# aosokin/os2d

Hardware: AMD Instinct MI355X
Metric: query-image-pairs/s (1280-px input, ResNet50, N-class) (higher is better)
Workload: dtype fftx3 (as fft; the per-bin complex GEMM on the fp16 MFMA with spectra split into fp16 hi+lo, 3 MFMAs per product, fp32 accumulate)

## Files before the change

os2d_amd/csrc/dft_mfma.h:

```cpp
#pragma once

#ifndef DFT_DEV
#error "the includer defines DFT_DEV, DFT_TID, DFT_BID, DFT_GRID, DFT_LDS, DFT_BARRIER, DFT_MFMA, DFT_SHFL_XOR, DFT_SHFL_XOR_U32, DFT_BALLOT, DFT_FLAG, DFT_FLAG_SET, DFT_RAISE, DFT_UNIFORM"
#endif

#ifndef DFT_MEMBER
#define DFT_MEMBER inline
#endif
#ifndef DFT_LANDED
#define DFT_LANDED(X)
#endif
#ifndef DFT_SWAP1
#define DFT_SWAP1(V) DFT_SHFL_XOR(V, 1)
#endif
#ifndef DFT_FWD_PREFETCH_AFTER
#define DFT_FWD_PREFETCH_AFTER 2
#endif
#ifndef DFT_INV_PREFETCH_AFTER
#define DFT_INV_PREFETCH_AFTER 2
#endif
#ifndef DFT_PIPE_REGA
#define DFT_PIPE_REGA 1
#endif
#ifndef DFT_PIPE_LDS
#define DFT_PIPE_LDS 1
#endif
#ifndef DFT_SCHED_FENCE
#define DFT_SCHED_FENCE()
#endif
#ifndef DFT_STREAM_STORE
#define DFT_STREAM_STORE(P, V) (*(P) = (V))
#endif
#ifndef DFT_STAMP
#define DFT_STAMP(K)
#define DFT_STAMP_BEGIN()
#define DFT_STAMP_END(BASE)
#endif

#include "tile_common.h"
#include "dft_plan.h"

namespace os2d_dft {

typedef float f32x4u __attribute__((ext_vector_type(4), aligned(4)));

DFT_DEV int dft_div(int x, unsigned magic) { return magic ? (int)(((unsigned long long)(unsigned)x * magic) >> 32) : x; }

DFT_DEV void dft_split4(float a, float b, float c, float d, u32x2* hi, u32x2* lo) {
  const f32x4 x = {a, b, c, d};
  const half4 h = __builtin_convertvector(x, half4);
  *hi = __builtin_bit_cast(u32x2, h);
#ifdef DFT_SPLIT_LO_PAIR
  u32x2 l;
  l[0] = DFT_SPLIT_LO_PAIR(a, b, (*hi)[0]);
  l[1] = DFT_SPLIT_LO_PAIR(c, d, (*hi)[1]);
  *lo = l;
#else
  const half4 l = __builtin_convertvector(x - __builtin_convertvector(h, f32x4), half4);
  *lo = __builtin_bit_cast(u32x2, l);
#endif
}

DFT_DEV half8 dft_frag(const u32x4* p) { return __builtin_bit_cast(half8, *p); }

DFT_DEV f32x16 dft_mma3(half8 ah, half8 al, half8 bh, half8 bl, f32x16 acc) {
  acc = DFT_MFMA(ah, bl, acc);
  acc = DFT_MFMA(al, bh, acc);
  acc = DFT_MFMA(ah, bh, acc);
  return acc;
}

template <int NT, int KS>
DFT_DEV void dft_product_rega(f32x16* acc, const half8* ah, const half8* al, int ksn, const u32x4* B, int bstride, int nt0,
                              int ntstep, int l31, int hw) {
  constexpr int KR = KS ? KS : DFT_KREG;
  half8 bh[2][NT], bl[2][NT];
#define DFT_REGA_READ(KSTEP, SET)                                                                                          \
  _Pragma("unroll") for (int j = 0; j < NT; ++j) {                                                                         \
    bh[SET][j] = dft_frag(B + (size_t)((2 * (KSTEP) + hw) * 2 + 0) * bstride + (nt0 + ntstep * j) * 32 + l31);             \
    bl[SET][j] = dft_frag(B + (size_t)((2 * (KSTEP) + hw) * 2 + 1) * bstride + (nt0 + ntstep * j) * 32 + l31);             \
  }
  if (DFT_PIPE_REGA) DFT_REGA_READ(0, 0)
#pragma unroll
  for (int ks = 0; ks < KR; ++ks) {
    if (KS || ks < ksn) {
      if (DFT_PIPE_REGA) {
        if (ks + 1 < KR && (KS || ks + 1 < ksn)) DFT_REGA_READ(ks + 1, (ks + 1) & 1)
        DFT_SCHED_FENCE();
      } else {
        DFT_REGA_READ(ks, ks & 1)
      }
#pragma unroll
      for (int j = 0; j < NT; ++j) acc[j] = dft_mma3(ah[ks], al[ks], bh[ks & 1][j], bl[ks & 1][j], acc[j]);
      if (DFT_PIPE_REGA) DFT_SCHED_FENCE();
    }
  }
#undef DFT_REGA_READ
}

template <int KS>
DFT_DEV void dft_product_rega_any(f32x16* acc, int ntiles, const half8* ah, const half8* al, int ksn, const u32x4* B, int bstride,
                                  int nt0, int ntstep, int l31, int hw) {
  if (ntiles == 3) dft_product_rega<3, KS>(acc, ah, al, ksn, B, bstride, nt0, ntstep, l31, hw);
  else if (ntiles == 2) dft_product_rega<2, KS>(acc, ah, al, ksn, B, bstride, nt0, ntstep, l31, hw);
  else if (ntiles == 1) dft_product_rega<1, KS>(acc, ah, al, ksn, B, bstride, nt0, ntstep, l31, hw);
}

template <int NT, bool SHARE, int NW, int PIPE_MODE>
DFT_DEV void dft_product_lds(f32x16* acc, int ks0, int ks1, const u32x4* A, int astride, const u32x4* B, int bstride, int t0, int mtn,
                             int l31, int hw) {
  constexpr int NA = SHARE ? 1 : NT;
  int tm[NT], tn[NT];
#pragma unroll
  for (int j = 0; j < NT; ++j) {
    const int t = t0 + NW * j;
    tn[j] = t / mtn;
    tm[j] = t - tn[j] * mtn;
  }
  half8 ah[2][NA], al[2][NA], bh[2][NT], bl[2][NT];
#define DFT_LDS_READ(KSTEP, SET)                                                                                           \
  {                                                                                                                        \
    const int kc_ = (KSTEP) < ks1 ? (KSTEP) : ks1 - 1;                                                                     \
    _Pragma("unroll") for (int j = 0; j < NA; ++j) {                                                                       \
      ah[SET][j] = dft_frag(A + (size_t)((2 * kc_ + hw) * 2 + 0) * astride + tm[j] * 32 + l31);                            \
      al[SET][j] = dft_frag(A + (size_t)((2 * kc_ + hw) * 2 + 1) * astride + tm[j] * 32 + l31);                            \
    }                                                                                                                      \
    _Pragma("unroll") for (int j = 0; j < NT; ++j) {                                                                       \
      bh[SET][j] = dft_frag(B + (size_t)((2 * kc_ + hw) * 2 + 0) * bstride + tn[j] * 32 + l31);                            \
      bl[SET][j] = dft_frag(B + (size_t)((2 * kc_ + hw) * 2 + 1) * bstride + tn[j] * 32 + l31);                            \
    }                                                                                                                      \
  }
#define DFT_LDS_MMA(SET)                                                                                                   \
  DFT_SCHED_FENCE();                                                                                                       \
  _Pragma("unroll") for (int j = 0; j < NT; ++j)                                                                           \
    acc[j] = dft_mma3(ah[SET][SHARE ? 0 : j], al[SET][SHARE ? 0 : j], bh[SET][j], bl[SET][j], acc[j]);                    \
  DFT_SCHED_FENCE();
  if (ks0 >= ks1) return;
  constexpr bool PIPE = PIPE_MODE == 2 || (PIPE_MODE == 1 && SHARE);
  if (!PIPE) {
    for (int ks = ks0; ks < ks1; ++ks) {
      DFT_LDS_READ(ks, 0)
      _Pragma("unroll") for (int j = 0; j < NT; ++j)
        acc[j] = dft_mma3(ah[0][SHARE ? 0 : j], al[0][SHARE ? 0 : j], bh[0][j], bl[0][j], acc[j]);
    }
    return;
  }
  DFT_LDS_READ(ks0, 0)
  int ks = ks0;
  for (; ks + 1 < ks1; ks += 2) {
    DFT_LDS_READ(ks + 1, 1)
    DFT_LDS_MMA(0)
    DFT_LDS_READ(ks + 2, 0)
    DFT_LDS_MMA(1)
  }
  if (ks < ks1) {
    DFT_LDS_MMA(0)
  }
#undef DFT_LDS_READ
#undef DFT_LDS_MMA
}

template <int NW, int PIPE_MODE>
DFT_DEV void dft_product_lds_any(f32x16* acc, int ntiles, int ks0, int ks1, const u32x4* A, int astride, const u32x4* B, int bstride,
                                 int t0, int mtn, int l31, int hw) {
  const bool share = mtn == NW;
  if (ntiles == 3) {
    if (share) dft_product_lds<3, true, NW, PIPE_MODE>(acc, ks0, ks1, A, astride, B, bstride, t0, mtn, l31, hw);
    else dft_product_lds<3, false, NW, PIPE_MODE>(acc, ks0, ks1, A, astride, B, bstride, t0, mtn, l31, hw);
  } else if (ntiles == 2) {
    if (share) dft_product_lds<2, true, NW, PIPE_MODE>(acc, ks0, ks1, A, astride, B, bstride, t0, mtn, l31, hw);
    else dft_product_lds<2, false, NW, PIPE_MODE>(acc, ks0, ks1, A, astride, B, bstride, t0, mtn, l31, hw);
  } else if (ntiles == 1) {
    dft_product_lds<1, true, NW, PIPE_MODE>(acc, ks0, ks1, A, astride, B, bstride, t0, mtn, l31, hw);
  }
}

DFT_DEV void dft_matrix_unit(int which, int unit, int P, int Q, const double* twP, const double* twQ, u32x4* out) {
  const int V = Q / 2 + 1;
  const bool r2 = which == 1 && dft_radix2(P);
  if (r2 && unit >= DFT_R2_MATU) {
    const int u = 2 * (unit - DFT_R2_MATU);
    u32x4 o;
    for (int t = 0; t < 4; ++t) o[t] = __builtin_bit_cast(unsigned, (float)twP[2 * u + t]);
    *out = o;
    return;
  }
  const int tws = r2 ? 2 : 1;
  if (r2) P /= 2;
  const int Pp = dft_round_up(P, 8);
  int cols, kidx, hl, col;
  double vals[8];
  if (which == 0) cols = dft_round_up(2 * V, 32);
  else if (which == 1 || which == 2) cols = dft_round_up(2 * P, 32);
  else cols = dft_round_up(Q, 32);
  col = unit % cols;
  hl = (unit / cols) & 1;
  kidx = unit / (2 * cols);
  for (int t = 0; t < 8; ++t) {
    const int k = kidx * 8 + t;
    double x = 0.0;
    if (which == 0) {
      const int v = col >> 1, ri = col & 1;
      if (k < Q && v < V) x = twQ[2 * (int)(((long long)v * k) % Q) + ri] * DFT_SCALE_F;
    } else if (r2) {
      const int h = 8 * (2 * (kidx >> 1) + (t >> 2)) + 4 * (kidx & 1) + (t & 3), u = col & 31;
      if (kidx < 4) {
        const int a = (int)(((long long)u * h) % P) * tws;
        x = (col < 32 ? twP[2 * a] : -twP[2 * a + 1]) * DFT_SCALE_F;
      }
    } else if (which == 1) {
      const int ri = k / Pp, h = k - ri * Pp, u = col >> 1, ro = col & 1;
      if (h < P && u < P && ri < 2) {
        const int a = (int)(((long long)u * h) % P) * tws;
        const double c = twP[2 * a], s = -twP[2 * a + 1];
        x = (ro == 0 ? (ri == 0 ? c : s) : (ri == 0 ? -s : c)) * DFT_SCALE_F;
      }
    } else if (which == 2) {
      const int ri = k / Pp, u = k - ri * Pp, h = col >> 1, ro = col & 1;
      if (u < P && h < P && ri < 2) {
        const int a = (int)(((long long)u * h) % P);
        const double c = twP[2 * a], s = -twP[2 * a + 1];
        x = (ro == 0 ? (ri == 0 ? c : -s) : (ri == 0 ? s : c)) * DFT_SCALE_F;
      }
    } else {
      const int v = k >> 1, ri = k & 1;
      if (v < V && col < Q) {
        const double a = (v == 0 || 2 * v == Q) ? 1.0 : 2.0;
        x = a * twQ[2 * (int)(((long long)v * col) % Q) + ri] * DFT_SCALE_GQ;
      }
    }
    vals[t] = x;
  }
  unsigned w[4];
  for (int t = 0; t < 4; ++t) {
    unsigned short b[2];
    for (int e = 0; e < 2; ++e) {
      const double x = vals[2 * t + e];
      const _Float16 h = (_Float16)x;
      const _Float16 r = hl == 0 ? h : (_Float16)(x - (double)h);
      b[e] = __builtin_bit_cast(unsigned short, r);
    }
    w[t] = (unsigned)b[0] | ((unsigned)b[1] << 16);
  }
  u32x4 o;
  o[0] = w[0];
  o[1] = w[1];
  o[2] = w[2];
  o[3] = w[3];
  *out = o;
}

template <bool TILED, bool FAST, int G, int NW, int KS2 = 0>
DFT_DEV void dft_forward_body(const float* corr,
                              const float* invn,
                              float* X,
                              const u32x4* FqT, const u32x4* Fp2, const DftPlan& pl, int C, int Cpad, int NBT, int iters) {
  constexpr int THR = NW * 64;
  constexpr bool ALDS = G == 8;
  constexpr bool R2 = !ALDS && KS2 == DFT_R2_KS;
  unsigned char* smem = DFT_LDS;
  const int tid = DFT_TID, lane = tid & 63, l31 = lane & 31, hw = lane >> 5;
  const int wv = DFT_UNIFORM(tid >> 6);
  const int P = pl.P, V = pl.V, Pp = pl.Pp, Wk = pl.Wk, N1 = pl.N1, Mx = pl.Mx, N2 = pl.N2, LH = pl.LH, LW = pl.LW, W = pl.W, H = pl.H;
  const int MxS = dft_pitch_x(pl), N2S = dft_pitch_n2(pl);
  const int CG = (C + G - 1) / G, HW = H * W;
  const bool unit_norm = invn == nullptr;
  u32x4* ldsF = reinterpret_cast<u32x4*>(smem);
  u32x4* ldsU = reinterpret_cast<u32x4*>(smem + pl.lds_const);
  unsigned char* ldsUb = smem + pl.lds_const;
  const int nF = dft_lds_fqt(pl);
  for (int i = tid; i < nF; i += THR) ldsF[i] = FqT[i];
  const unsigned char* ldsTw = dft_lds_tail_ptr(smem, pl) + DFT_TAIL_TW;
  if (R2 && tid < DFT_R2_TWU) reinterpret_cast<u32x4*>(dft_lds_tail_ptr(smem, pl) + DFT_TAIL_TW)[tid] = Fp2[DFT_R2_MATU + tid];
  u32x4* ldsP = ldsF + nF;
  if (ALDS)
    for (int i = tid; i < dft_lds_rowop(Pp, pl.M2); i += THR) ldsP[i] = Fp2[i];

  const int mt1n = Mx / 32, nt1n = N1 / 32, nt2n = N2 / 32, mt2n = pl.M2 / 32;
  const int ks1n = Wk / 16, ks2n = 2 * Pp / 16;
  const int mt2 = wv & 3;
  constexpr int KR2 = R2 ? 4 : KS2 ? KS2 : DFT_KREG;
  half8 fp2h[KR2], fp2l[KR2];
  if (R2) {
#pragma unroll
    for (int f = 0; f < KR2; ++f) {
      fp2h[f] = dft_frag(Fp2 + ((size_t)((2 * (f & 1) + hw) * 2 + 0)) * 64 + (f >> 1) * 32 + l31);
      fp2l[f] = dft_frag(Fp2 + ((size_t)((2 * (f & 1) + hw) * 2 + 1)) * 64 + (f >> 1) * 32 + l31);
    }
  } else if (!ALDS) {
#pragma unroll
    for (int ks = 0; ks < KR2; ++ks) {
      const int kc = ks < ks2n ? ks : 0, mc = mt2 < mt2n ? mt2 : 0;
      fp2h[ks] = dft_frag(Fp2 + ((size_t)((2 * kc + hw) * 2 + 0)) * pl.M2 + mc * 32 + l31);
      fp2l[ks] = dft_frag(Fp2 + ((size_t)((2 * kc + hw) * 2 + 1)) * pl.M2 + mc * 32 + l31);
    }
  }
  if (!ALDS) {
#pragma unroll
    for (int ks = 0; ks < KR2; ++ks) {
// ... 216 lines not shown

      const int XS = dft_pitch_xs(P, G);
#pragma unroll
      for (int j = 0; j < DFT_ACC_TILES; ++j) {
        if (un[j] < 0) continue;
        const int n2 = un[j] * 32 + l31;
        const int img = dft_div(n2, pl.inv_v), v = n2 - img * V;
#pragma unroll
        for (int q = 0; q < 4; ++q) {
          const int u0 = (um[j] * 32 + 8 * q + 4 * hw) >> 1;
          if (img < G && u0 < P) {
            const float sc = DFT_SCALE_XOUT;
            f32x4 o;
            o[0] = xc[j][4 * q] * sc;
            o[1] = xc[j][4 * q + 1] * sc;
            o[2] = xc[j][4 * q + 2] * sc;
            o[3] = xc[j][4 * q + 3] * sc;
            *reinterpret_cast<f32x4*>(ldsUb + (size_t)v * XS + (u0 >> 2) * (G * 32) + img * 32 + (u0 & 3) * 8) = o;
          }
        }
      }
      DFT_BARRIER();
      DFT_STAMP(4)
    }

    {
      const int XS = dft_pitch_xs(P, G);
      const int per_v = (P / 4) * (G * 2), npieces = V * per_v;
      size_t qstride;
      float* dstbase = X + dft_spectra_pair0(pr_, NBT, pl.NBINS / 4, Cpad, &qstride) + (size_t)c0_ * 8;
      if (R2) {
        constexpr int per_h = (DFT_R2_P / 8) * (G * 2);
        for (int i = tl; i < V * per_h; i += THR) {
          const int v = i / per_h, rem = i - v * per_h;
          const int uq = rem / (2 * G), jj = rem - uq * (2 * G);
          const unsigned char* src = ldsUb + (size_t)v * XS + uq * (G * 32) + jj * 16;
          const f32x4 e = *reinterpret_cast<const f32x4*>(src);
          const f32x4 o = *reinterpret_cast<const f32x4*>(src + (DFT_R2_P / 8) * (G * 32));
          const f32x4 w = *reinterpret_cast<const f32x4*>(ldsTw + (4 * uq + 2 * (jj & 1)) * 8);
          f32x4 t;
          t[0] = w[0] * o[0] - w[1] * o[1];
          t[1] = w[0] * o[1] + w[1] * o[0];
          t[2] = w[2] * o[2] - w[3] * o[3];
          t[3] = w[2] * o[3] + w[3] * o[2];
          float* dst = dstbase + (size_t)(v * (P / 4) + uq) * qstride + jj * 4;
          DFT_STREAM_STORE(reinterpret_cast<f32x4*>(dst), e + t);
          DFT_STREAM_STORE(reinterpret_cast<f32x4*>(dst + (size_t)(DFT_R2_P / 8) * qstride), e - t);
        }
      } else
      for (int i = tl; i < npieces; i += THR) {
        const int v = dft_div(i, pl.inv_pq), rem = i - v * per_v;
        const int uq = rem / (2 * G), jj = rem - uq * (2 * G);
        const f32x4 val = *reinterpret_cast<const f32x4*>(ldsUb + (size_t)v * XS + uq * (G * 32) + jj * 16);
        DFT_STREAM_STORE(reinterpret_cast<f32x4*>(dstbase + (size_t)(v * (P / 4) + uq) * qstride + jj * 4), val);
      }
      const int qpad0 = (P * V) / 4, qpad1 = pl.NBINS / 4;
      for (int i = tl; i < (qpad1 - qpad0) * 2 * G; i += THR)
        *reinterpret_cast<f32x4*>(dstbase + (size_t)(qpad0 + i / (2 * G)) * qstride + (i % (2 * G)) * 4) = f32x4{0.f, 0.f, 0.f, 0.f};
    }
    DFT_BARRIER();
    DFT_STAMP(5)
  }
  DFT_STAMP_END(0)
#undef DFT_FWD_ITER
#undef DFT_FWD_POS
#undef DFT_FWD_PREFETCH
#undef DFT_FWD_PREFETCH_SLOTS
}

template <bool TILED, int KSA = 0, int G = DFT_G>
DFT_DEV void dft_inverse_body(const float* Y,
                              const float* bp,
                              int MTP, unsigned char* out,
                              const u32x4* E2, const u32x4* Gq, const DftPlan& pl, int Cout, int NBT, int PLANE, int Ws,
                              int BASE, int iters, DFT_FLAG bad_flag, int zero_borders) {
  unsigned char* smem = DFT_LDS;
  const int tid = DFT_TID, lane = tid & 63, l31 = lane & 31, hw = lane >> 5;
  const int wv = DFT_UNIFORM(tid >> 6);
  const int P = pl.P, V = pl.V, Pp = pl.Pp, N2 = pl.N2, MB = pl.MB, KB = pl.KB, NBo = pl.NBo, H = pl.H, W = pl.W;
  const int N2S = dft_pitch_n2(pl), MBS = dft_pitch_tt(pl);
  const int OG = Cout / G;
  constexpr bool ALDS = G == 8;
  constexpr int LG = G == 8 ? 3 : 2;
  u32x4* ldsG = reinterpret_cast<u32x4*>(smem);
  u32x4* ldsU = reinterpret_cast<u32x4*>(smem + pl.lds_const);
  unsigned char* ldsUb = smem + pl.lds_const;
  float* smaxw = reinterpret_cast<float*>(dft_lds_tail_ptr(smem, pl) + DFT_TAIL_MAX);
  const int nG = dft_lds_gq(pl), NQ = dft_round_up(pl.Q, 32);
  for (int i = tid; i < nG; i += DFT_THR) {
    const int kh = i / NBo, n = i - kh * NBo;
    ldsG[i] = Gq[(size_t)kh * NQ + n];
  }
  const int MAfull = dft_round_up(2 * P, 32);
  u32x4* ldsE = ldsG + nG;
  if (ALDS)
    for (int i = tid; i < dft_lds_rowop(Pp, MAfull); i += DFT_THR) ldsE[i] = E2[i];

  const int mtAn = pl.MA / 32, ntAn = N2 / 32, ksAn = 2 * Pp / 16;
  const int mtBn = MB / 32, ntBn = NBo / 32, ksBn = KB / 16;
  const int mtA = wv & 3;
  constexpr int KRA = KSA ? KSA : DFT_KREG;
  half8 e2h[KRA], e2l[KRA];
  if (!ALDS) {
#pragma unroll
    for (int ks = 0; ks < KRA; ++ks) {
      const int kc = ks < ksAn ? ks : 0, mc = mtA < mtAn ? mtA : 0;
      e2h[ks] = dft_frag(E2 + ((size_t)((2 * kc + hw) * 2 + 0)) * MAfull + mc * 32 + l31);
      e2l[ks] = dft_frag(E2 + ((size_t)((2 * kc + hw) * 2 + 1)) * MAfull + mc * 32 + l31);
    }
#pragma unroll
    for (int ks = 0; ks < KRA; ++ks) {
      DFT_LANDED(e2h[ks]);
      DFT_LANDED(e2l[ks]);
    }
  }

  constexpr int NITEM = DFT_ITEMS;
  const int uoct = Pp / 8, nitem = G * V * uoct;
  f32x4 py[NITEM][4];
#define DFT_INV_PREFETCH(IT, TID) DFT_INV_PREFETCH_ITEMS(IT, TID, 0, NITEM)
#define DFT_INV_PREFETCH_ITEMS(IT, TID, S0, S1)                                             \
  {                                                                                         \
    const int pr_ = dft_div((IT), pl.inv_og), og_ = (IT)-pr_ * OG;                          \
    size_t qstride;                                                                         \
    const float* src_ = Y + dft_spectra_pair0(pr_, NBT, pl.NBINS / 4, Cout, &qstride) + (size_t)og_ * G * 8; \
    _Pragma("unroll") for (int s = (S0); s < (S1); ++s) {                                   \
      const int e_ = (TID) + s * DFT_THR;                                                   \
      const int ec_ = e_ < nitem ? e_ : 0;                                                  \
      const int pimg_ = ec_ & (G - 1), prest_ = ec_ >> LG;                                  \
      const int pv_ = dft_div(prest_, pl.inv_kg), puo_ = prest_ - pv_ * (Pp / 8);           \
      const int q0_ = pv_ * (P / 4) + 2 * puo_;                                             \
      const bool ptwo_ = 8 * puo_ + 4 < P;                                                  \
      const float* p0_ = src_ + (size_t)q0_ * qstride + pimg_ * 8;                          \
      const float* p1_ = src_ + (size_t)(ptwo_ ? q0_ + 1 : q0_) * qstride + pimg_ * 8;      \
      py[s][0] = *reinterpret_cast<const f32x4*>(p0_);                                     \
      py[s][1] = *reinterpret_cast<const f32x4*>(p0_ + 4);                                 \
      py[s][2] = *reinterpret_cast<const f32x4*>(p1_);                                     \
      py[s][3] = *reinterpret_cast<const f32x4*>(p1_ + 4);                                 \
    }                                                                                       \
  }
#define DFT_INV_ITEM(E)                                                                     \
  const int img_ = (E) & (G - 1), rest_ = (E) >> LG;                                        \
  const int v_ = dft_div(rest_, pl.inv_kg), uo_ = rest_ - v_ * uoct;                        \
  const bool two_ = 8 * uo_ + 4 < P;
#define DFT_INV_MAXIMA(TID)                                                                 \
  {                                                                                         \
    float m = 0.f;                                                                          \
    _Pragma("unroll") for (int s = 0; s < NITEM; ++s)                                       \
      if ((TID) + s * DFT_THR < nitem) {                                                    \
        DFT_INV_ITEM((TID) + s * DFT_THR)                                                   \
        (void)img_;                                                                         \
        (void)v_;                                                                           \
        (void)uo_;                                                                          \
        _Pragma("unroll") for (int k = 0; k < 4; ++k)                                       \
          if (k < 2 || two_) {                                                              \
            _Pragma("unroll") for (int e = 0; e < 4; ++e) m = fmaxf(m, fabsf(py[s][k][e])); \
          }                                                                                 \
      }                                                                                     \
    if (G == 4) m = fmaxf(m, DFT_SHFL_XOR(m, 4));                                           \
    m = fmaxf(m, DFT_SHFL_XOR(m, 8));                                                       \
    m = fmaxf(m, DFT_SHFL_XOR(m, 16));                                                      \
    m = fmaxf(m, DFT_SHFL_XOR(m, 32));                                                      \
    if (lane < G) smaxw[wv * G + lane] = m;                                                 \
  }
  bool bad = false;
  const int first = (DFT_GRID & 7) == 0 ? (DFT_BID & 7) * (DFT_GRID >> 3) + (DFT_BID >> 3) : DFT_BID;
  if (first < iters) {
    DFT_INV_PREFETCH(first, tid)
    DFT_INV_MAXIMA(tid)
  }
  DFT_BARRIER();

  DFT_STAMP_BEGIN()
  for (int it = first; it < iters; it += DFT_GRID) {
    int tl = tid;
#ifndef OS2D_HOST_EMU
    asm volatile("" : "+v"(tl));
#endif
    const int lane = tl & 63, l31 = lane & 31, hw = lane >> 5;
    const int pr = dft_div(it, pl.inv_og), og = it - pr * OG;
    const int nb = TILED ? dft_div(pr, pl.inv_t) : pr, tile = TILED ? pr - nb * pl.T : 0;
    const int ty = TILED ? dft_div(tile, pl.inv_tx) : 0, tx = TILED ? tile - ty * pl.TX : 0;
    const int y0 = TILED ? ty * pl.TH : 0, x0 = TILED ? tx * pl.TW : 0, oy = TILED ? pl.oy : 0, ox = TILED ? pl.ox : 0;
    const int TH_ = TILED ? pl.TH : H, TW_ = TILED ? pl.TW : W;
    const int o0 = og * G;

    DFT_STAMP(0)
    float simg = 1.f, cinv[4] = {0.f, 0.f, 0.f, 0.f};
    {
#pragma unroll
      for (int g = 0; g < G; ++g) {
        float m = 0.f;
#pragma unroll
        for (int w = 0; w < DFT_WAVES; ++w) m = fmaxf(m, smaxw[w * G + g]);
        int E = (int)((__builtin_bit_cast(unsigned, m) >> 23) & 0xffu) - 127;
        if (!(m > 0.f) || E < -100) E = -100;
        if (E > 100) E = 100;
        const float s = __builtin_bit_cast(float, (unsigned)(DFT_EY - E + 127) << 23);
        const float sinv = __builtin_bit_cast(float, (unsigned)(E - DFT_EY + 127) << 23);
        if (g == (tl & (G - 1))) simg = s;
        const float ci = sinv * __builtin_bit_cast(float, (unsigned)(pl.eT - DFT_EGQ + 127) << 23) / (float)(P * pl.Q);
        if (G == 4 || (g >> 2) == hw) cinv[g & 3] = ci;
      }
    }
#pragma unroll
    for (int s = 0; s < NITEM; ++s) {
      const int e = tl + s * DFT_THR;
      if (e < nitem) {
        DFT_INV_ITEM(e)
        const int img = img_, v = v_, uo = uo_;
        const bool two = two_;
        float re[8], im[8];
#pragma unroll
        for (int k = 0; k < 4; ++k) {
          const bool ok = k < 2 || two;
          re[2 * k] = ok ? py[s][k][0] * simg : 0.f;
          im[2 * k] = ok ? py[s][k][1] * simg : 0.f;
          re[2 * k + 1] = ok ? py[s][k][2] * simg : 0.f;
          im[2 * k + 1] = ok ? py[s][k][3] * simg : 0.f;
        }
        u32x2 h0, l0, h1, l1;
        u32x4 t;
        const size_t n = (size_t)img * V + v;
        dft_split4(re[0], re[1], re[2], re[3], &h0, &l0);
        dft_split4(re[4], re[5], re[6], re[7], &h1, &l1);
        t[0] = h0[0], t[1] = h0[1], t[2] = h1[0], t[3] = h1[1];
        ldsU[(size_t)((uo)*2 + 0) * N2S + n] = t;
        t[0] = l0[0], t[1] = l0[1], t[2] = l1[0], t[3] = l1[1];
        ldsU[(size_t)((uo)*2 + 1) * N2S + n] = t;
        dft_split4(im[0], im[1], im[2], im[3], &h0, &l0);
        dft_split4(im[4], im[5], im[6], im[7], &h1, &l1);
        t[0] = h0[0], t[1] = h0[1], t[2] = h1[0], t[3] = h1[1];
        ldsU[(size_t)((uoct + uo) * 2 + 0) * N2S + n] = t;
        t[0] = l0[0], t[1] = l0[1], t[2] = l1[0], t[3] = l1[1];
        ldsU[(size_t)((uoct + uo) * 2 + 1) * N2S + n] = t;
      }
    }
    DFT_BARRIER();
    DFT_STAMP(1)

    f32x16 ta[DFT_ACC_TILES];
    int an[DFT_ACC_TILES], am[DFT_ACC_TILES];
    int ntaw = 0;
#pragma unroll
    for (int j = 0; j < DFT_ACC_TILES; ++j) {
      const int t = wv + DFT_WAVES * j;
      const int nt = ALDS ? t / mtAn : (wv >> 2) + 2 * j;
      const bool mine = ALDS ? t < mtAn * ntAn : (nt < ntAn && mtA < mtAn);
      an[j] = mine ? nt : -1;
      am[j] = ALDS ? t - nt * mtAn : mtA;
      ntaw += mine ? 1 : 0;
#pragma unroll
      for (int r = 0; r < 16; ++r) ta[j][r] = 0.f;
    }
    const int itn = it + DFT_GRID < iters ? it + DFT_GRID : it;
    {
      if (ALDS) {
        dft_product_lds_any<DFT_WAVES, DFT_PIPE_LDS ? 1 : 0>(ta, ntaw, 0, ksAn, ldsE, MAfull, ldsU, N2S, wv, mtAn, l31, hw);
        DFT_INV_PREFETCH_ITEMS(itn, tl, 0, NITEM)
      } else if (DFT_INV_PREFETCH_AFTER == 1 || (DFT_INV_PREFETCH_AFTER == 2 && KSA > 0 && KSA <= 6)) {
        dft_product_rega_any<KSA>(ta, ntaw, e2h, e2l, ksAn, ldsU, N2S, wv >> 2, 2, l31, hw);
        DFT_INV_PREFETCH_ITEMS(itn, tl, 0, NITEM)
      } else {
        DFT_INV_PREFETCH_ITEMS(itn, tl, 0, NITEM)
        dft_product_rega_any<KSA>(ta, ntaw, e2h, e2l, ksAn, ldsU, N2S, wv >> 2, 2, l31, hw);
      }
    }
    DFT_BARRIER();
    DFT_STAMP(2)

    {
      const float sc = __builtin_bit_cast(float, (unsigned)(127 - DFT_EF - pl.eT) << 23);
#pragma unroll
      for (int j = 0; j < DFT_ACC_TILES; ++j) {
        if (an[j] < 0) continue;
        const int n = an[j] * 32 + l31;
        const int img = dft_div(n, pl.inv_v), v = n - img * V;
        if (img >= G) continue;
#pragma unroll
        for (int q = 0; q < 4; ++q) {
          const int h0 = (am[j] * 32 + 8 * q + 4 * hw) >> 1;
          u32x2 hi, lo;
          dft_split4(ta[j][4 * q] * sc, ta[j][4 * q + 1] * sc, ta[j][4 * q + 2] * sc, ta[j][4 * q + 3] * sc, &hi, &lo);
          unsigned char* d0 = ldsUb + ((size_t)((v >> 2) * 2) * MBS + (size_t)h0 * G + img) * 16 + (v & 3) * 4;
          *reinterpret_cast<unsigned*>(d0) = hi[0];
          *reinterpret_cast<unsigned*>(d0 + (size_t)MBS * 16) = lo[0];
          *reinterpret_cast<unsigned*>(d0 + G * 16) = hi[1];
          *reinterpret_cast<unsigned*>(d0 + G * 16 + (size_t)MBS * 16) = lo[1];
        }
      }
      for (int v = V; v < KB / 2; ++v)
        for (int m = tl; m < MB; m += DFT_THR) {
          unsigned char* d0 = ldsUb + ((size_t)((v >> 2) * 2) * MBS + m) * 16 + (v & 3) * 4;
          *reinterpret_cast<unsigned*>(d0) = 0u;
          *reinterpret_cast<unsigned*>(d0 + (size_t)MBS * 16) = 0u;
        }
    }
    DFT_BARRIER();
    DFT_STAMP(3)

    f32x16 yc[DFT_ACC_TILES];
    int bm[DFT_ACC_TILES], bn[DFT_ACC_TILES];
    int ntbw = 0;
#pragma unroll
    for (int j = 0; j < DFT_ACC_TILES; ++j) {
      const int t = wv + DFT_WAVES * j;
      const bool mine = t < mtBn * ntBn;
      bn[j] = mine ? t / mtBn : 0;
      bm[j] = mine ? t - bn[j] * mtBn : -1;
      ntbw += mine ? 1 : 0;
#pragma unroll
      for (int r = 0; r < 16; ++r) yc[j][r] = 0.f;
    }
    dft_product_lds_any<DFT_WAVES, DFT_PIPE_LDS ? 1 : 0>(yc, ntbw, 0, ksBn, ldsU, MBS, ldsG, NBo, wv, mtBn, l31, hw);
    DFT_INV_MAXIMA(tl)
    DFT_STAMP(4)

    {
      const bool planes = zero_borders == DFT_OUT_PLANES;
      float bias[4], osc[4];
#pragma unroll
      for (int g = 0; g < 4; ++g) {
        bias[g] = bp[o0 + (G == 8 ? 4 * hw : 0) + g];
        osc[g] = bp[2 * MTP + o0 + (G == 8 ? 4 * hw : 0) + g];
      }
      const int grp = o0 >> 3, slot = o0 & 7;
      unsigned char* hi_unit = out + (((size_t)nb * ((Cout + 7) >> 3) + grp) * 2 + 0) * (size_t)PLANE * 16 + slot * 2;
      unsigned char* lo_unit = out + (((size_t)nb * ((Cout + 7) >> 3) + grp) * 2 + 1) * (size_t)PLANE * 16 + slot * 2;
      if (zero_borders == DFT_OUT_SHB_BORDERS && (!TILED || tile == 0)) {
        const int rows = H * (Ws - W), tail0 = BASE + H * Ws, npad = BASE + rows + (PLANE - tail0);
        for (int k = tl; k < npad; k += DFT_THR) {
          int cell;
          if (k < BASE) cell = k;
          else if (k < BASE + rows) {
            const int jj = k - BASE, hr = jj / (Ws - W);
            cell = BASE + hr * Ws + W + (jj - hr * (Ws - W));
          } else cell = tail0 + (k - BASE - rows);
          if (G == 8) {
            *reinterpret_cast<u32x4*>(hi_unit + (size_t)cell * 16) = u32x4{0u, 0u, 0u, 0u};
            *reinterpret_cast<u32x4*>(lo_unit + (size_t)cell * 16) = u32x4{0u, 0u, 0u, 0u};
          } else {
            *reinterpret_cast<u32x2*>(hi_unit + (size_t)cell * 16) = u32x2{0u, 0u};
            *reinterpret_cast<u32x2*>(lo_unit + (size_t)cell * 16) = u32x2{0u, 0u};
          }
        }
      }
#pragma unroll
      for (int j = 0; j < DFT_ACC_TILES; ++j) {
        if (bm[j] < 0) continue;
        const int wwin = bn[j] * 32 + l31, tw = wwin - ox;
#pragma unroll
        for (int q = 0; q < 4; ++q) {
          const int hwin = G == 8 ? bm[j] * 4 + q : (bm[j] * 32 + 8 * q + 4 * hw) >> 2, th = hwin - oy;
          const int h = y0 + th, w = x0 + tw;
          const bool inside = th >= 0 && th < TH_ && tw >= 0 && tw < TW_ && h < H && w < W;
          if (G == 8 || inside) {
            float t[4];
#pragma unroll
            for (int g = 0; g < 4; ++g) {
              const float pre = yc[j][4 * q + g] * cinv[g] + bias[g];
              t[g] = fmaxf(pre, 0.f) * osc[g];
              if (inside && (!(fabsf(t[g]) <= 65504.f) || pre != pre)) bad = true;
            }
            if (planes) {
              if (inside) {
                float* dst = reinterpret_cast<float*>(out) + ((size_t)nb * Cout + o0 + (G == 8 ? 4 * hw : 0)) * ((size_t)H * W) + (size_t)h * W + w;
#pragma unroll
                for (int g = 0; g < 4; ++g) dst[(size_t)g * H * W] = t[g] * DFT_SCALE_PLANES;
              }
              continue;
            }
            u32x2 hi, lo;
            dft_split4(t[0], t[1], t[2], t[3], &hi, &lo);
            const size_t off = ((size_t)BASE + (size_t)h * Ws + w) * 16;
// ... 30 lines not shown
```

os2d_amd/csrc/dft_plan.h:

```cpp
#pragma once

#include <stddef.h>
#include <stdlib.h>

#ifndef DFT_HD
#define DFT_HD static inline
#endif

namespace os2d_dft {

constexpr int DFT_THR = 512, DFT_WAVES = 8;
constexpr int DFT_G = 4;
constexpr int DFT_MAXP = 64;
constexpr int DFT_MAXV = 48;
constexpr int DFT_MAXWK = 96;
constexpr int DFT_KREG = 8;
constexpr int DFT_LDS_MAX = 160 * 1024;
constexpr int DFT_OUT_SHB = 0, DFT_OUT_SHB_BORDERS = 1, DFT_OUT_PLANES = 2;

constexpr int DFT_ACC_TILES = 3;
constexpr int DFT_SLOTS_G4 = 3, DFT_SLOTS_G8 = 2;
constexpr int DFT_ITEMS = 3;

constexpr int DFT_EX = 15;
constexpr int DFT_EF = 14;
constexpr int DFT_EGQ = 13;
constexpr int DFT_ER = 8;
constexpr int DFT_EY = 13;
constexpr double dft_pow2(int e) { return e >= 0 ? (double)(1 << e) : 1.0 / (double)(1 << -e); }
constexpr float DFT_SCALE_X = (float)dft_pow2(DFT_EX);
constexpr double DFT_SCALE_F = dft_pow2(DFT_EF), DFT_SCALE_GQ = dft_pow2(DFT_EGQ);
constexpr float DFT_SCALE_R = (float)dft_pow2(DFT_ER - DFT_EX - DFT_EF);
constexpr float DFT_SCALE_XOUT = (float)dft_pow2(-(DFT_ER + DFT_EF));
constexpr float DFT_SCALE_PLANES = (float)dft_pow2(-DFT_EX);

struct DftPlan {
  int H, W;
  int P, Q, V, NBINS;
  int T, TY, TX, TH, TW;
  int oy, ox;
  int LH, LW;
  int RH;
  int Pp;
  int Wk;
  int N1;
  int M2;
  int Mx;
  int N2;
  int MA;
  int MB;
  int KB;
  int NBo;
  int G;
  int eT;
  int fast;
  unsigned inv_cg, inv_t, inv_tx, inv_c4, inv_v, inv_pq, inv_og, inv_kg, inv_pp;
  int lds_const, lds_union, lds_total;
};

DFT_HD constexpr int dft_round_up(int x, int m) { return (x + m - 1) / m * m; }
DFT_HD unsigned dft_magic(unsigned d) { return d > 1 ? (unsigned)(((1ull << 32) + d - 1) / d) : 0u; }

DFT_HD int dft_units_fqt(int P, int Q) { return (dft_round_up(Q, 16) / 8) * 2 * dft_round_up(Q + 2, 32); }
constexpr int DFT_R2_P = 64, DFT_R2_MATU = 8 * 2 * 64, DFT_R2_TWU = 16;
DFT_HD bool dft_radix2(int P) { return P == DFT_R2_P; }
DFT_HD int dft_units_fp2(int P, int Q) {
  return dft_radix2(P) ? DFT_R2_MATU + DFT_R2_TWU : (2 * dft_round_up(P, 8) / 8) * 2 * dft_round_up(2 * P, 32);
}
DFT_HD int dft_units_e2(int P, int Q) { return (2 * dft_round_up(P, 8) / 8) * 2 * dft_round_up(2 * P, 32); }
DFT_HD int dft_units_gq(int P, int Q) { return (dft_round_up(Q + 2, 16) / 8) * 2 * dft_round_up(Q, 32); }
DFT_HD size_t dft_matrices_units(int P, int Q) {
  return (size_t)dft_units_fqt(P, Q) + dft_units_fp2(P, Q) + dft_units_e2(P, Q) + dft_units_gq(P, Q);
}

DFT_HD int dft_lds_units(int k, int pitch) { return (k / 8) * 2 * pitch; }
DFT_HD int dft_lds_fqt(const DftPlan& pl) { return dft_lds_units(pl.Wk, pl.N1); }
DFT_HD int dft_lds_gq(const DftPlan& pl) { return dft_lds_units(pl.KB, pl.NBo); }
DFT_HD int dft_lds_rowop(int Pp, int rows) { return dft_lds_units(2 * Pp, rows); }
DFT_HD int dft_pitch_x(const DftPlan& pl) { return pl.Mx + 1; }
DFT_HD int dft_pitch_n2(const DftPlan& pl) { return pl.N2 + 1; }
DFT_HD int dft_pitch_tt(const DftPlan& pl) { return pl.MB + 1; }
DFT_HD int dft_pitch_xs(int P, int G) { return P * 8 * G + 16; }
DFT_HD int dft_lds_x_bytes(const DftPlan& pl) { return dft_lds_units(pl.Wk, dft_pitch_x(pl)) * 16; }
DFT_HD int dft_lds_n2_bytes(const DftPlan& pl) { return dft_lds_units(2 * pl.Pp, dft_pitch_n2(pl)) * 16; }
DFT_HD int dft_lds_xs_bytes(const DftPlan& pl, int G) { return pl.V * dft_pitch_xs(pl.P, G); }
DFT_HD int dft_lds_tt_bytes(const DftPlan& pl) { return dft_lds_units(pl.KB, dft_pitch_tt(pl)) * 16; }
constexpr int DFT_TAIL_BYTES = 1024;
constexpr int DFT_TAIL_MAX = 0, DFT_TAIL_TW = 512;
constexpr int dft_tail_max_bytes(int G) { return DFT_WAVES * G * 4; }
static_assert(DFT_TAIL_MAX + dft_tail_max_bytes(8) <= DFT_TAIL_TW, "the maxima of 8 images end in front of the twiddles");
static_assert(DFT_TAIL_TW + DFT_R2_TWU * 16 <= DFT_TAIL_BYTES, "the twiddles end inside the tail");
DFT_HD int dft_lds_tail(const DftPlan& pl) { return pl.lds_const + pl.lds_union; }
DFT_HD unsigned char* dft_lds_tail_ptr(unsigned char* smem, const DftPlan& pl) { return smem + pl.lds_const + pl.lds_union; }

struct DftCounts {
  int t1, t2, tA, tB;
  int rows2, cols2;
  int npos, nitem;
};
DFT_HD DftCounts dft_plan_counts(const DftPlan& pl) {
  DftCounts c;
  c.t1 = (pl.Mx / 32) * (pl.N1 / 32);
  c.t2 = (pl.M2 / 32) * (pl.N2 / 32);
  c.tA = (pl.MA / 32) * (pl.N2 / 32);
  c.tB = (pl.MB / 32) * (pl.NBo / 32);
  c.rows2 = (pl.M2 > pl.MA ? pl.M2 : pl.MA) / 32;
  c.cols2 = pl.N2 / 32;
  c.npos = pl.Pp * (pl.Wk / 4);
  c.nitem = pl.G * pl.V * (pl.Pp / 8);
  return c;
}
DFT_HD bool dft_capacity_ok(const DftPlan& pl) {
  const DftCounts c = dft_plan_counts(pl);
  const int tiles = DFT_WAVES * DFT_ACC_TILES;
  if (c.t1 > tiles || c.tB > tiles || c.nitem > DFT_ITEMS * DFT_THR) return false;
  if (pl.G == 8) return c.t2 <= tiles && c.tA <= tiles && c.npos <= DFT_SLOTS_G8 * DFT_THR;
  return c.rows2 <= 4 && c.cols2 <= (DFT_WAVES / 4) * DFT_ACC_TILES && c.npos <= DFT_SLOTS_G4 * DFT_THR;
}
static_assert(dft_round_up(DFT_G * DFT_MAXP, 32) / 32 <= DFT_WAVES && dft_round_up(2 * DFT_MAXV, 32) / 32 <= DFT_ACC_TILES,
              "step 1: at most 8 x 3 tiles");
static_assert(dft_round_up(2 * DFT_MAXP, 32) / 32 <= 4 && dft_round_up(DFT_G * DFT_MAXV, 32) / 32 <= (DFT_WAVES / 4) * DFT_ACC_TILES,
              "step 2 / step A: at most 4 row tiles, 6 column tiles reached as (wave >> 2) + 2 j");
static_assert(DFT_G * (dft_round_up(2 * DFT_MAXP, 32) / 2) / 32 <= DFT_WAVES && dft_round_up(DFT_MAXWK, 32) / 32 <= DFT_ACC_TILES,
              "step B: at most 8 x 3 tiles");
static_assert(dft_round_up(DFT_MAXP, 8) * (DFT_MAXWK / 4) <= DFT_SLOTS_G4 * DFT_THR, "window positions: at most 64 * 24");
static_assert(DFT_G * DFT_MAXV * (dft_round_up(DFT_MAXP, 8) / 8) <= DFT_ITEMS * DFT_THR, "spectrum items: at most 4 * 48 * 8");
static_assert(2 * dft_round_up(DFT_MAXP, 8) / 16 <= DFT_KREG, "k-steps of the register-resident operand");

static inline bool dft_plan_transform(int LH, int LW, int RH, int ncols, int minP, int minQ, int G, DftPlan* pl) {
  pl->G = G;
  pl->P = dft_round_up(minP, 4);
  if (pl->P == 60) pl->P = DFT_R2_P;
  pl->Q = dft_round_up(minQ, 2);
  pl->V = pl->Q / 2 + 1;
  pl->NBINS = dft_round_up(pl->P * pl->V, 8);
  pl->LH = LH;
  pl->LW = LW;
  pl->RH = RH;
  pl->Pp = dft_round_up(pl->P, 8);
  pl->Wk = dft_round_up(LW, 16);
  pl->N1 = dft_round_up(2 * pl->V, 32);
  pl->M2 = dft_round_up(2 * pl->P, 32);
  pl->Mx = dft_round_up(G * pl->Pp, 32);
  pl->N2 = dft_round_up(G * pl->V, 32);
  pl->MA = dft_round_up(2 * RH, 32);
  pl->MB = G * (pl->MA / 2);
  pl->KB = dft_round_up(2 * pl->V, 16);
  pl->NBo = dft_round_up(ncols, 32);
  int e = 0;
  while ((1 << e) < pl->P) ++e;
  pl->eT = e + 1;
  if (pl->P > DFT_MAXP || pl->V > DFT_MAXV || pl->Wk > DFT_MAXWK || LH > pl->P || LW > pl->Q || RH > pl->P) return false;
// ... 103 lines not shown
```

Measured before the change: 51830.

## Use radix-2 even/odd split for the P=64 inverse DFT stage

For P=64 the inverse stage now does a radix-2 decimation instead of a dense complex DFT GEMM. It multiplies even- and odd-indexed halves by a half-size 32-point DFT matrix held in registers, then combines them with twiddles staged in LDS to write both output halves. This is meant to cut MFMA work and the register footprint of the E2 matrix, at the cost of more epilogue arithmetic and a new matrix layout. It also zeroes the padded spectrum rows with wide vector stores instead of per-word stores.

```diff
diff --git a/os2d_amd/csrc/dft_mfma.h b/os2d_amd/csrc/dft_mfma.h
--- a/os2d_amd/csrc/dft_mfma.h
+++ b/os2d_amd/csrc/dft_mfma.h
@@ -18,6 +18,9 @@
 #endif
 #ifndef DFT_INV_PREFETCH_AFTER
 #define DFT_INV_PREFETCH_AFTER 2
+#endif
+#ifndef DFT_INV_ZERO_WIDE
+#define DFT_INV_ZERO_WIDE 1
 #endif
 #ifndef DFT_PIPE_REGA
 #define DFT_PIPE_REGA 1
@@ -106,6 +109,35 @@
   else if (ntiles == 1) dft_product_rega<1, KS>(acc, ah, al, ksn, B, bstride, nt0, ntstep, l31, hw);
 }
 
+template <int NT>
+DFT_DEV void dft_product_rega_eo(f32x16* e, f32x16* o, const half8* ah, const half8* al, const u32x4* B, int bstride, int nt0,
+                                 int ntstep, int l31, int hw) {
+  constexpr int KR = DFT_R2_KS / 2;
+  half8 bh[2][2][NT], bl[2][2][NT];
+#define DFT_EO_READ(KSTEP, SET)                                                                                            \
+  _Pragma("unroll") for (int p = 0; p < 2; ++p) _Pragma("unroll") for (int j = 0; j < NT; ++j) {                           \
+    bh[SET][p][j] = dft_frag(B + (size_t)((2 * ((KSTEP) + KR * p) + hw) * 2 + 0) * bstride + (nt0 + ntstep * j) * 32 + l31); \
+    bl[SET][p][j] = dft_frag(B + (size_t)((2 * ((KSTEP) + KR * p) + hw) * 2 + 1) * bstride + (nt0 + ntstep * j) * 32 + l31); \
+  }
+  if (DFT_PIPE_REGA) DFT_EO_READ(0, 0)
+#pragma unroll
+  for (int ks = 0; ks < KR; ++ks) {
+    if (DFT_PIPE_REGA) {
+      if (ks + 1 < KR) DFT_EO_READ(ks + 1, (ks + 1) & 1)
+      DFT_SCHED_FENCE();
+    } else {
+      DFT_EO_READ(ks, ks & 1)
+    }
+#pragma unroll
+    for (int j = 0; j < NT; ++j) {
+      e[j] = dft_mma3(ah[ks], al[ks], bh[ks & 1][0][j], bl[ks & 1][0][j], e[j]);
+      o[j] = dft_mma3(ah[ks], al[ks], bh[ks & 1][1][j], bl[ks & 1][1][j], o[j]);
+    }
+    if (DFT_PIPE_REGA) DFT_SCHED_FENCE();
+  }
+#undef DFT_EO_READ
+}
+
 template <int NT, bool SHARE, int NW, int PIPE_MODE>
 DFT_DEV void dft_product_lds(f32x16* acc, int ks0, int ks1, const u32x4* A, int astride, const u32x4* B, int bstride, int t0, int mtn,
                              int l31, int hw) {
@@ -177,16 +209,16 @@
 
 DFT_DEV void dft_matrix_unit(int which, int unit, int P, int Q, const double* twP, const double* twQ, u32x4* out) {
   const int V = Q / 2 + 1;
-  const bool r2 = which == 1 && dft_radix2(P);
-  if (r2 && unit >= DFT_R2_MATU) {
-    const int u = 2 * (unit - DFT_R2_MATU);
+  const bool r2 = which == 1 && dft_radix2(P), r2i = which == 2 && dft_radix2_inv(P);
+  if ((r2 && unit >= DFT_R2_MATU) || (r2i && unit >= DFT_R2I_MATU)) {
+    const int u = 2 * (unit - (r2 ? DFT_R2_MATU : DFT_R2I_MATU));
     u32x4 o;
-    for (int t = 0; t < 4; ++t) o[t] = __builtin_bit_cast(unsigned, (float)twP[2 * u + t]);
+    for (int t = 0; t < 4; ++t) o[t] = __builtin_bit_cast(unsigned, (float)(r2i && (t & 1) ? -twP[2 * u + t] : twP[2 * u + t]));
     *out = o;
     return;
   }
-  const int tws = r2 ? 2 : 1;
-  if (r2) P /= 2;
+  const int tws = r2 || r2i ? 2 : 1;
+  if (r2 || r2i) P /= 2;
   const int Pp = dft_round_up(P, 8);
   int cols, kidx, hl, col;
   double vals[8];
@@ -215,6 +247,11 @@
         const double c = twP[2 * a], s = -twP[2 * a + 1];
         x = (ro == 0 ? (ri == 0 ? c : s) : (ri == 0 ? -s : c)) * DFT_SCALE_F;
       }
+    } else if (r2i) {
+      const int ri = t >> 2, m = 4 * kidx + (t & 3), h = col >> 1, ro = col & 1;
+      const int a = (int)(((long long)m * h) % P) * tws;
+      const double c = twP[2 * a], s = -twP[2 * a + 1];
+      x = (ro == 0 ? (ri == 0 ? c : -s) : (ri == 0 ? s : c)) * DFT_SCALE_F;
     } else if (which == 2) {
       const int ri = k / Pp, u = k - ri * Pp, h = col >> 1, ro = col & 1;
       if (u < P && h < P && ri < 2) {
@@ -597,6 +634,12 @@
   const int OG = Cout / G;
   constexpr bool ALDS = G == 8;
   constexpr int LG = G == 8 ? 3 : 2;
+  constexpr bool R2I = !ALDS && KSA == DFT_R2_KS && dft_radix2_inv(DFT_R2_P);
+  const unsigned char* ldsTw = dft_lds_tail_ptr(smem, pl) + DFT_TAIL_TW;
+  if (R2I && tid < DFT_R2_TWU) {
+    const f32x4 w = __builtin_bit_cast(f32x4, E2[DFT_R2I_MATU + tid]);
+    reinterpret_cast<f32x4*>(dft_lds_tail_ptr(smem, pl) + DFT_TAIL_TW)[tid] = w * __builtin_bit_cast(float, (unsigned)(127 - DFT_EF - pl.eT) << 23);
+  }
   u32x4* ldsG = reinterpret_cast<u32x4*>(smem);
   u32x4* ldsU = reinterpret_cast<u32x4*>(smem + pl.lds_const);
   unsigned char* ldsUb = smem + pl.lds_const;
@@ -613,10 +656,21 @@
 
   const int mtAn = pl.MA / 32, ntAn = N2 / 32, ksAn = 2 * Pp / 16;
   const int mtBn = MB / 32, ntBn = NBo / 32, ksBn = KB / 16;
-  const int mtA = wv & 3;
-  constexpr int KRA = KSA ? KSA : DFT_KREG;
+  const int mtA = R2I ? wv & 1 : wv & 3;
+  constexpr int KRA = R2I ? KSA / 2 : KSA ? KSA : DFT_KREG;
   half8 e2h[KRA], e2l[KRA];
-  if (!ALDS) {
+  if (R2I) {
+#pragma unroll
+    for (int ks = 0; ks < KRA; ++ks) {
+      e2h[ks] = dft_frag(E2 + ((size_t)((2 * ks + hw) * 2 + 0)) * 64 + mtA * 32 + l31);
+      e2l[ks] = dft_frag(E2 + ((size_t)((2 * ks + hw) * 2 + 1)) * 64 + mtA * 32 + l31);
+    }
+#pragma unroll
+    for (int ks = 0; ks < KRA; ++ks) {
+      DFT_LANDED(e2h[ks]);
+      DFT_LANDED(e2l[ks]);
+    }
+  } else if (!ALDS) {
 #pragma unroll
     for (int ks = 0; ks < KRA; ++ks) {
       const int kc = ks < ksAn ? ks : 0, mc = mtA < mtAn ? mtA : 0;
@@ -737,14 +791,14 @@
         u32x2 h0, l0, h1, l1;
         u32x4 t;
         const size_t n = (size_t)img * V + v;
-        dft_split4(re[0], re[1], re[2], re[3], &h0, &l0);
-        dft_split4(re[4], re[5], re[6], re[7], &h1, &l1);
+        if (R2I) dft_split4(re[0], re[2], re[4], re[6], &h0, &l0), dft_split4(im[0], im[2], im[4], im[6], &h1, &l1);
+        else dft_split4(re[0], re[1], re[2], re[3], &h0, &l0), dft_split4(re[4], re[5], re[6], re[7], &h1, &l1);
         t[0] = h0[0], t[1] = h0[1], t[2] = h1[0], t[3] = h1[1];
         ldsU[(size_t)((uo)*2 + 0) * N2S + n] = t;
         t[0] = l0[0], t[1] = l0[1], t[2] = l1[0], t[3] = l1[1];
         ldsU[(size_t)((uo)*2 + 1) * N2S + n] = t;
-        dft_split4(im[0], im[1], im[2], im[3], &h0, &l0);
-        dft_split4(im[4], im[5], im[6], im[7], &h1, &l1);
+        if (R2I) dft_split4(re[1], re[3], re[5], re[7], &h0, &l0), dft_split4(im[1], im[3], im[5], im[7], &h1, &l1);
+        else dft_split4(im[0], im[1], im[2], im[3], &h0, &l0), dft_split4(im[4], im[5], im[6], im[7], &h1, &l1);
         t[0] = h0[0], t[1] = h0[1], t[2] = h1[0], t[3] = h1[1];
         ldsU[(size_t)((uoct + uo) * 2 + 0) * N2S + n] = t;
         t[0] = l0[0], t[1] = l0[1], t[2] = l1[0], t[3] = l1[1];
@@ -760,17 +814,26 @@
 #pragma unroll
     for (int j = 0; j < DFT_ACC_TILES; ++j) {
       const int t = wv + DFT_WAVES * j;
-      const int nt = ALDS ? t / mtAn : (wv >> 2) + 2 * j;
-      const bool mine = ALDS ? t < mtAn * ntAn : (nt < ntAn && mtA < mtAn);
+      const int nt = R2I ? (wv >> 1) + 4 * j : ALDS ? t / mtAn : (wv >> 2) + 2 * j;
+      const bool mine = R2I ? (j < 2 && nt < ntAn && 32 * mtA < pl.MA) : ALDS ? t < mtAn * ntAn : (nt < ntAn && mtA < mtAn);
       an[j] = mine ? nt : -1;
       am[j] = ALDS ? t - nt * mtAn : mtA;
       ntaw += mine ? 1 : 0;
 #pragma unroll
       for (int r = 0; r < 16; ++r) ta[j][r] = 0.f;
     }
+    f32x16 tb[DFT_ACC_TILES];
+#pragma unroll
+    for (int j = 0; j < DFT_ACC_TILES; ++j)
+#pragma unroll
+      for (int r = 0; r < 16; ++r) tb[j][r] = 0.f;
     const int itn = it + DFT_GRID < iters ? it + DFT_GRID : it;
     {
-      if (ALDS) {
+      if constexpr (R2I) {
+        DFT_INV_PREFETCH_ITEMS(itn, tl, 0, NITEM)
+        if (ntaw == 2) dft_product_rega_eo<2>(ta, tb, e2h, e2l, ldsU, N2S, wv >> 1, 4, l31, hw);
+        else if (ntaw == 1) dft_product_rega_eo<1>(ta, tb, e2h, e2l, ldsU, N2S, wv >> 1, 4, l31, hw);
+      } else if (ALDS) {
         dft_product_lds_any<DFT_WAVES, DFT_PIPE_LDS ? 1 : 0>(ta, ntaw, 0, ksAn, ldsE, MAfull, ldsU, N2S, wv, mtAn, l31, hw);
         DFT_INV_PREFETCH_ITEMS(itn, tl, 0, NITEM)
       } else if (DFT_INV_PREFETCH_AFTER == 1 || (DFT_INV_PREFETCH_AFTER == 2 && KSA > 0 && KSA <= 6)) {
@@ -792,6 +855,36 @@
         const int n = an[j] * 32 + l31;
         const int img = dft_div(n, pl.inv_v), v = n - img * V;
         if (img >= G) continue;
+        if constexpr (R2I) {
+          const int MAh = pl.MA / 2;
+#pragma unroll
+          for (int q = 0; q < 4; ++q) {
+            const int h0 = 16 * mtA + 4 * q + 2 * hw;
+            const f32x4 w = *reinterpret_cast<const f32x4*>(ldsTw + h0 * 8);
+            const float e0 = ta[j][4 * q], e1 = ta[j][4 * q + 1], e2 = ta[j][4 * q + 2], e3 = ta[j][4 * q + 3];
+            const float o0 = tb[j][4 * q], o1 = tb[j][4 * q + 1], o2 = tb[j][4 * q + 2], o3 = tb[j][4 * q + 3];
+            const float t0 = w[0] * o0 - w[1] * o1, t1 = w[0] * o1 + w[1] * o0;
+            const float t2 = w[2] * o2 - w[3] * o3, t3 = w[2] * o3 + w[3] * o2;
+            unsigned char* d0 = ldsUb + ((size_t)((v >> 2) * 2) * MBS + (size_t)h0 * G + img) * 16 + (v & 3) * 4;
+            u32x2 hi, lo;
+            if (h0 < MAh) {
+              dft_split4(e0 * sc + t0, e1 * sc + t1, e2 * sc + t2, e3 * sc + t3, &hi, &lo);
+              *reinterpret_cast<unsigned*>(d0) = hi[0];
+              *reinterpret_cast<unsigned*>(d0 + (size_t)MBS * 16) = lo[0];
+              *reinterpret_cast<unsigned*>(d0 + G * 16) = hi[1];
+              *reinterpret_cast<unsigned*>(d0 + G * 16 + (size_t)MBS * 16) = lo[1];
+            }
+            if (h0 + 32 < MAh) {
+              unsigned char* d1 = d0 + 32 * G * 16;
+              dft_split4(e0 * sc - t0, e1 * sc - t1, e2 * sc - t2, e3 * sc - t3, &hi, &lo);
+              *reinterpret_cast<unsigned*>(d1) = hi[0];
+              *reinterpret_cast<unsigned*>(d1 + (size_t)MBS * 16) = lo[0];
+              *reinterpret_cast<unsigned*>(d1 + G * 16) = hi[1];
+              *reinterpret_cast<unsigned*>(d1 + G * 16 + (size_t)MBS * 16) = lo[1];
+            }
+          }
+          continue;
+        }
 #pragma unroll
         for (int q = 0; q < 4; ++q) {
           const int h0 = (am[j] * 32 + 8 * q + 4 * hw) >> 1;
@@ -804,7 +897,17 @@
           *reinterpret_cast<unsigned*>(d0 + G * 16 + (size_t)MBS * 16) = lo[1];
         }
       }
-      for (int v = V; v < KB / 2; ++v)
+      int vnarrow = KB / 2;
+      if constexpr (R2I && DFT_INV_ZERO_WIDE) {
+        vnarrow = (V + 3) & ~3;
+        if (vnarrow > KB / 2) vnarrow = KB / 2;
+        for (int vq = vnarrow >> 2; vq < KB / 8; ++vq)
+          for (int m = tl; m < MB; m += DFT_THR) {
+            ldsU[(size_t)(vq * 2) * MBS + m] = u32x4{0u, 0u, 0u, 0u};
+            ldsU[(size_t)(vq * 2 + 1) * MBS + m] = u32x4{0u, 0u, 0u, 0u};
+          }
+      }
+      for (int v = V; v < vnarrow; ++v)
         for (int m = tl; m < MB; m += DFT_THR) {
           unsigned char* d0 = ldsUb + ((size_t)((v >> 2) * 2) * MBS + m) * 16 + (v & 3) * 4;
           *reinterpret_cast<unsigned*>(d0) = 0u;
diff --git a/os2d_amd/csrc/dft_plan.h b/os2d_amd/csrc/dft_plan.h
--- a/os2d_amd/csrc/dft_plan.h
+++ b/os2d_amd/csrc/dft_plan.h
@@ -67,7 +67,17 @@
 DFT_HD int dft_units_fp2(int P, int Q) {
   return dft_radix2(P) ? DFT_R2_MATU + DFT_R2_TWU : (2 * dft_round_up(P, 8) / 8) * 2 * dft_round_up(2 * P, 32);
 }
-DFT_HD int dft_units_e2(int P, int Q) { return (2 * dft_round_up(P, 8) / 8) * 2 * dft_round_up(2 * P, 32); }
+constexpr int DFT_R2I_MATU = 8 * 2 * 64;
+DFT_HD constexpr bool dft_radix2_inv(int P) {
+#ifdef DFT_INV_DENSE64
+  return false;
+#else
+  return P == DFT_R2_P;
+#endif
+}
+DFT_HD int dft_units_e2(int P, int Q) {
+  return dft_radix2_inv(P) ? DFT_R2I_MATU + DFT_R2_TWU : (2 * dft_round_up(P, 8) / 8) * 2 * dft_round_up(2 * P, 32);
+}
 DFT_HD int dft_units_gq(int P, int Q) { return (dft_round_up(Q + 2, 16) / 8) * 2 * dft_round_up(Q, 32); }
 DFT_HD size_t dft_matrices_units(int P, int Q) {
   return (size_t)dft_units_fqt(P, Q) + dft_units_fp2(P, Q) + dft_units_e2(P, Q) + dft_units_gq(P, Q);
```

After: 51460. About the same (-0.7%).
